# barronalex/Tacotron

Measured on AMD Instinct MI355X. Metric: mel-frames/sec (train step, batch=32 r=2), higher is better.
Workload: dtype f32

## Files before the change

### include/taco_hip.h

```cpp
#ifndef TACO_HIP_H
#define TACO_HIP_H

#include <stddef.h>
#include <stdint.h>

#ifdef __cplusplus
extern "C" {
#endif
#pragma GCC visibility push(default)

#define TACO_VERSION 120

#define TACO_OK 0
#define TACO_EINVAL (-1)
#define TACO_ELAUNCH (-2)
#define TACO_ENOTFOUND (-3)

#define TACO_ACT_NONE 0
#define TACO_ACT_RELU 1
#define TACO_ACT_SIGMOID 2
#define TACO_ACT_TANH 3

typedef struct TacoShape {
  int32_t B;
  int32_t Tt;
  int32_t Td;
  int32_t r;
  int32_t V;
  int32_t S;
} TacoShape;

typedef struct TacoTensorInfo {
  char name[64];
  int64_t offset;
  int64_t size;
  int32_t ndim;
  int32_t dims[4];
} TacoTensorInfo;

int taco_version(void);
const char* taco_last_error_string(void);

int64_t taco_param_count(const TacoShape* shape);
int taco_param_table(const TacoShape* shape, TacoTensorInfo* rows, int cap);

int64_t taco_workspace_bytes(const TacoShape* shape, int train);
int taco_workspace_table(const TacoShape* shape, int train, TacoTensorInfo* rows, int cap);

int taco_conv_gemm(const float* A, int lda, const float* W, int ldw, const float* bias, const float* scale,
                   const float* shift, const float* residual, int ldr, const uint8_t* keep, float* C, int ldc,
                   float* Cpre, int M, int N, int K, int taps, int T, int pad_l, int act, void* stream);

int taco_debug_gemm2_window(int lo, int hi);
int64_t taco_debug_weight_image(const float* W, int ldw, int taps, int K, int N, void* img, int64_t img_bytes, void* stream);
int taco_debug_conv_gemm_nld(const float* A, int lda, const float* W, int ldw, int nld, const float* bias, float* C, int ldc, int M,
                             int N, int K, int act, void* stream);
int taco_debug_conv_gemm_ksplit(const float* A, int lda, const float* W, int ldw, const float* bias, float* C, int ldc, int M,
                                int N, int K, int taps, int T, int pad_l, int act, float* slabs, int64_t slab_floats,
                                void* stream);

int taco_gemm_tn(const float* A, int lda, const float* dY, int ldy, float* dW, int ldw, int M, int N, int K, int taps,
                 int T, int pad_l, int accumulate, void* stream);

int taco_debug_gemm_naive(const float* A, int lda, const float* W, int ldw, const float* bias, float* C, int ldc,
                          int M, int N, int K, int taps, int T, int pad_l, int act, void* stream);

int taco_bigru_fwd(const float* x, const float* wg_fw, const float* bg_fw, const float* wc_fw, const float* bc_fw,
                   const float* wg_bw, const float* bg_bw, const float* wc_bw, const float* bc_bw, float* xg,
                   float* out, float* ruc, int B, int T, void* stream);

int taco_debug_bigru_rec_fwd(const float* xg, const float* wg_fw, const float* wc_fw, const float* wg_bw, const float* wc_bw,
                             const float* h0, float* out, float* ruc, int B, int T, void* stream);
int taco_debug_bigru_bwd(const float* dout, const float* out, const float* ruc, const float* wghT_fw, const float* wchT_fw,
                         const float* wghT_bw, const float* wchT_bw, const float* h0, float* dxg, float* rh, float* dh0, int B, int T,
                         void* stream);
int taco_debug_highway_stack_fwd(const float* x, const float* const* wt, const float* const* bt, const float* const* wh,
                                 const float* const* bh, float* const* th, float* const* y, const float* const* wa,
                                 const float* const* rowb, float* const* hx, int M, int nl, int T, void* stream);
int taco_debug_highway_stack_bwd(const float* g, const float* const* wT, const float* const* th, const float* const* x,
                                 float* const* dth, float* gout, const float* const* waT, float* const* dhx, int M, int nl, void* stream);
int taco_debug_prenet_fwd(const float* x, const float* w1, const float* b1, const float* w2, const float* b2, const uint8_t* keep1,
                          const uint8_t* keep2, float* y1, float* y2, int M, void* stream);
int taco_debug_prenet_bwd(const float* dy2, const float* w2T, const float* w1T, const uint8_t* keep1, const uint8_t* keep2,
                          const float* y1_in, const float* y2_in, float* dz2, float* dz1, float* dx, int M, void* stream);

int taco_debug_conv_bank_pool_fwd(const float* x, int lda, const float* const* W, const float* const* bias, const float* scale,
                                  const float* shift, float scale_mul, float* pool, float* bank, int ldc, int M, int T, int F, int N, int K,
                                  void* stream);
int taco_debug_conv_gemm_pool_bwd(const float* A, int lda, const float* W, int ldw, const float* pool_x, const float* scale,
                                  const float* shift, float scale_mul, float* C, int ldc, float* dgamma, float* dbeta, int M, int N, int K,
                                  int taps, int T, int pad_l, void* stream);
int taco_debug_bn_maxpool_fwd(const float* x, const float* gamma, const float* beta, float* y, int B, int T, int C, void* stream);
int taco_debug_bn_maxpool_bwd(const float* x, const float* gamma, const float* beta, const float* dy, float* dx, float* dgamma,
                              float* dbeta, int B, int T, int C, void* stream);
int taco_debug_bank_gather(const float* dbank, int lda, const float* const* WT, const float* residual, int ldr, float* dx_out, int ldc,
                           float* slabs, int64_t slab_floats, int M, int T, int F, int K, int N, int pad_l, int S, void* stream);
int taco_debug_conv_gemm_batch_atomic(const float* dbank, int lda, const float* const* WT, const float* residual, int ldr, float* dx_out,
                                      int ldc, int M, int T, int F, int K, int N, void* stream);
int taco_debug_conv_gemm_rowbias(const float* A, int lda, const float* W, int ldw, const float* rowb, int bias_stride, float* C, int ldc,
                                 int M, int T, int N, int K, void* stream);
int taco_debug_gemm_tn_group(int n, const float* const* A, const int* lda, const float* const* Y, const int* ldy, float* const* W,
                             const int* ldw, float* const* dbias, const int* M, const int* N, const int* K, const int* taps,
                             const int* T, const int* pad_l, void* stream);
int taco_debug_gemm_tn_strided(const float* A, int lda, int64_t strideA, const float* Y, int ldy, int64_t strideY, float* W, int ldw,
                               int64_t strideW, int M, int N, int K, int T, int pad_l, int batch, void* stream);

// ... 213 lines not shown
```

### tacotron_amd/csrc/gemm.hip

```cpp
#include <algorithm>

#include "bf16x3.h"
#include "common.h"
#include "kernels.h"

namespace {

constexpr int BK = 16;

__device__ __forceinline__ float4 sel4(bool ok, const float4 t) {
  return make_float4(ok ? t.x : 0.f, ok ? t.y : 0.f, ok ? t.z : 0.f, ok ? t.w : 0.f);
}

struct RowInfo {
  int m;
  int t;
  bool ok;
};

template <int WM, int WN, bool VA, bool VB>
__global__ __launch_bounds__(256) void conv_gemm_kernel(ConvGemmBatch batch) {
  constexpr int BM = 64 * WM, BN = 64 * WN;
  constexpr int LDS_A = BM + 4, LDS_B = BN + 4;
  constexpr int A_PER = BM / 64;
// ... 176 lines not shown
        for (int e = 0; e < 16; ++e) {
          const int m = min(mrow + (e & 3) + 8 * (e >> 2), P.M - 1);
          res_e[e] = P.residual[(int64_t)m * P.ldr + n];
        }
      }
      float pre_e[16];
#pragma unroll
      for (int e = 0; e < 16; ++e) {
        float v = apply_act(acc[i][j][e] + bias_e[e], P.act);
        if (P.keep) v = keep_e[e] ? v * 2.0f : 0.0f;
        pre_e[e] = v;
        if (P.scale || P.shift) v = v * sc + sf;
        acc[i][j][e] = v + res_e[e];
      }
      __builtin_amdgcn_sched_barrier(0);
#pragma unroll
      for (int e = 0; e < 16; ++e) {
        const int m = mrow + (e & 3) + 8 * (e >> 2);
        if (m >= P.M) continue;
        if (P.Cpre) P.Cpre[(int64_t)m * P.ldc + n] = pre_e[e];
        if (P.atomic_out) atomicAdd(&P.C[(int64_t)m * P.ldc + n], acc[i][j][e]);
        else P.C[(int64_t)m * P.ldc + n] = acc[i][j][e];
      }
    }
  }
}

__global__ void conv_gemm_tapsum_kernel(ConvGemmProblem P, const float* __restrict__ slabs, int taps) {
  const int64_t total4 = (int64_t)P.M * P.N / 4;
  const int64_t slab = (int64_t)P.M * P.N;
  for (int64_t i = (int64_t)blockIdx.x * blockDim.x + threadIdx.x; i < total4; i += (int64_t)gridDim.x * blockDim.x) {
    const int m = (int)(i * 4 / P.N), n0 = (int)(i * 4 - (int64_t)m * P.N);
    float4 s = reinterpret_cast<const float4*>(slabs)[i];
    for (int t = 1; t < taps; ++t) {
      const float4 v = reinterpret_cast<const float4*>(slabs + t * slab)[i];
      s.x += v.x; s.y += v.y; s.z += v.z; s.w += v.w;
    }
    float r[4] = {s.x, s.y, s.z, s.w};
#pragma unroll
    for (int j = 0; j < 4; ++j) {
      const int n = n0 + j;
      const float bias = P.bias ? (P.bias_stride ? P.bias[(int64_t)(m / P.T) * P.bias_stride + n] : P.bias[n]) : 0.f;
      float v = apply_act(r[j] + bias, P.act);
      if (P.keep) v = P.keep[(int64_t)m * P.N + n] ? v * 2.0f : 0.0f;
      if (P.Cpre) P.Cpre[(int64_t)m * P.ldc + n] = v;
      if (P.scale || P.shift) v = v * (P.scale ? P.scale[n] * P.scale_mul : 1.f) + (P.shift ? P.shift[n] : 0.f);
      if (P.residual) v += P.residual[(int64_t)m * P.ldr + n];
      if (P.atomic_out) P.C[(int64_t)m * P.ldc + n] += v;
      else P.C[(int64_t)m * P.ldc + n] = v;
    }
  }
}

template <int WM, int WN, bool VA, bool VB, bool BX = false>
__device__ __forceinline__ void gemm_tn_body(const GemmTnArgs& P, const int bx, const int by, const int bz_) {
  constexpr int BM = 64 * WM, BN = 64 * WN;
  constexpr int LDS_A = BM + 4, LDS_B = BN + 4;
  constexpr int A_PER = BM / 64, B_PER = BN / 64;
  const int k0 = bx * BM, n0 = by * BN;
  int z = bz_;
  const int split = z % P.splits;
  z /= P.splits;
  const int tap = z % P.taps;
  const int bz = z / P.taps;
  const float* A = P.A + (int64_t)bz * P.strideA;
  const float* Y = P.Y + (int64_t)bz * P.strideY;
  float* W = P.W + (int64_t)bz * P.strideW + (int64_t)tap * P.K * P.ldw;

  __shared__ __attribute__((aligned(16))) float As[2][BK][LDS_A];
  __shared__ __attribute__((aligned(16))) float Bs[2][BK][LDS_B];

  const int tid = threadIdx.x, lane = tid & 63, wave = tid >> 6;
  const int wm = wave >> 1, wn = wave & 1;
  const int sh = tap - P.pad_l;

  constexpr int A_COLS4 = BM / 4, B_COLS4 = BN / 4;
  constexpr int A_RSTEP = 256 / A_COLS4, B_RSTEP = 256 / B_COLS4;
  const int a_c4 = tid % A_COLS4, a_r = tid / A_COLS4;
  const int b_c4 = tid % B_COLS4, b_r = tid / B_COLS4;

  const int m_begin = split * P.chunk;
  const int m_end = min(P.M, m_begin + P.chunk);
  const int nit = (m_end - m_begin + BK - 1) / BK;
  if (nit <= 0) return;

  float4 ra[A_PER], rb[B_PER];
  const bool do_bias = P.dbias != nullptr && bx == 0 && tap == 0;
  float4 bsum[B_PER];
#pragma unroll
  for (int i = 0; i < B_PER; ++i) bsum[i] = make_float4(0.f, 0.f, 0.f, 0.f);
  constexpr int kOOB = (int)0x80000000;
  __amdgpu_buffer_rsrc_t rsA, rsY;
  int a_vo[A_PER], a_t[A_PER], b_vo[B_PER];
  int sh_t = sh;
  if constexpr (VA) {
    int kcol = k0 + a_c4 * 4;
    if (P.ktap > 0) {
      const int tc = kcol / P.ktap;
      kcol -= tc * P.ktap;
      sh_t = tc - P.pad_l;
    }
    rsA = __builtin_amdgcn_make_buffer_rsrc(const_cast<float*>(A - (int64_t)16 * P.lda), 0, 0x7fffffff, 0x00020000);
#pragma unroll
    for (int i = 0; i < A_PER; ++i) {
      const int r = a_r + i * A_RSTEP, k = k0 + a_c4 * 4;
      a_vo[i] = (r < BK && k < P.K) ? ((m_begin + r + sh_t + 16) * P.lda + kcol) * 4 : kOOB;
      a_t[i] = (m_begin + r) % P.T;
    }
  }
  if constexpr (VB) {
    rsY = __builtin_amdgcn_make_buffer_rsrc(const_cast<float*>(Y), 0, 0x7fffffff, 0x00020000);
#pragma unroll
    for (int i = 0; i < B_PER; ++i) {
      const int r = b_r + i * B_RSTEP, n = n0 + b_c4 * 4;
      b_vo[i] = (r < BK && n < P.Nld) ? ((m_begin + r) * P.ldy + n) * 4 : kOOB;
    }
  }
  auto as_f4 = [](auto v) { return __builtin_bit_cast(float4, v); };
  auto load_tile = [&](int it) {
    const int mm0 = m_begin + it * BK;
#pragma unroll
    for (int i = 0; i < A_PER; ++i) {
      float4 v = make_float4(0.f, 0.f, 0.f, 0.f);
      const int r = a_r + i * A_RSTEP;
      const int m = mm0 + r;
      const int k = k0 + a_c4 * 4;
      if constexpr (VA) {
        const bool ok = m < m_end && (unsigned)(a_t[i] + sh_t) < (unsigned)P.T;
        v = as_f4(__builtin_amdgcn_raw_buffer_load_b128(rsA, ok ? a_vo[i] : kOOB, it * (BK * 4) * P.lda, 0));
        a_t[i] += BK;
        if (P.T >= BK) a_t[i] = a_t[i] >= P.T ? a_t[i] - P.T : a_t[i];
        else a_t[i] %= P.T;
      } else if (r < BK && m < m_end) {
        const int st = (m % P.T) + sh;
        if (st >= 0 && st < P.T) {
          const float* p = A + (int64_t)(m + sh) * P.lda + k;
          if (k < P.K) v.x = p[0];
          if (k + 1 < P.K) v.y = p[1];
          if (k + 2 < P.K) v.z = p[2];
          if (k + 3 < P.K) v.w = p[3];
        }
      }
      ra[i] = v;
    }
#pragma unroll
    for (int i = 0; i < B_PER; ++i) {
      float4 v = make_float4(0.f, 0.f, 0.f, 0.f);
      const int r = b_r + i * B_RSTEP;
      const int m = mm0 + r;
      const int n = n0 + b_c4 * 4;
      if constexpr (VB) {
        v = as_f4(__builtin_amdgcn_raw_buffer_load_b128(rsY, m < m_end ? b_vo[i] : kOOB, it * (BK * 4) * P.ldy, 0));
      } else if (r < BK && m < m_end) {
        const float* p = Y + (int64_t)m * P.ldy + n;
        if (n < P.N) v.x = p[0];
        if (n + 1 < P.N) v.y = p[1];
        if (n + 2 < P.N) v.z = p[2];
        if (n + 3 < P.N) v.w = p[3];
      }
      rb[i] = v;
    }
  };
  auto store_tile = [&](int buf) {
#pragma unroll
    for (int i = 0; i < A_PER; ++i) {
      const int r = a_r + i * A_RSTEP;
      if (r < BK) *reinterpret_cast<float4*>(&As[buf][r][a_c4 * 4]) = ra[i];
    }
#pragma unroll
    for (int i = 0; i < B_PER; ++i) {
      const int r = b_r + i * B_RSTEP;
      const float4 v = rb[i];
      if (r < BK) *reinterpret_cast<float4*>(&Bs[buf][r][b_c4 * 4]) = v;
      if (do_bias) { bsum[i].x += v.x; bsum[i].y += v.y; bsum[i].z += v.z; bsum[i].w += v.w; }
    }
  };

  f32x16 acc[WM][WN];
#pragma unroll
  for (int i = 0; i < WM; ++i)
#pragma unroll
    for (int j = 0; j < WN; ++j)
#pragma unroll
      for (int e = 0; e < 16; ++e) acc[i][j][e] = 0.f;
  f32x16 acc_lo[BX ? WM : 1][BX ? WN : 1];
#pragma unroll
  for (int i = 0; i < (BX ? WM : 1); ++i)
#pragma unroll
    for (int j = 0; j < (BX ? WN : 1); ++j)
#pragma unroll
      for (int e = 0; e < 16; ++e) acc_lo[i][j][e] = 0.f;

  load_tile(0);
  store_tile(0);
  __syncthreads();
  const int lk = lane >> 5, li = lane & 31;
  for (int it = 0; it < nit; ++it) {
    const int buf = it & 1;
    if (it + 1 < nit) load_tile(it + 1);
    if constexpr (BX) {
      static_assert(BK == 16, "one v_mfma_f32_32x32x16_bf16 group per 16-row tile");
      Pl3 pa[WM], pb[WN];
#pragma unroll
      for (int i = 0; i < WM; ++i) {
        float f[8];
#pragma unroll
        for (int q = 0; q < 8; ++q) f[q] = As[buf][2 * q + lk][wm * (32 * WM) + i * 32 + li];
        pa[i] = split8(f[0], f[1], f[2], f[3], f[4], f[5], f[6], f[7]);
      }
#pragma unroll
      for (int j = 0; j < WN; ++j) {
        float f[8];
#pragma unroll
        for (int q = 0; q < 8; ++q) f[q] = Bs[buf][2 * q + lk][wn * (32 * WN) + j * 32 + li];
        pb[j] = split8(f[0], f[1], f[2], f[3], f[4], f[5], f[6], f[7]);
      }
#pragma unroll
      for (int i = 0; i < WM; ++i)
#pragma unroll
        for (int j = 0; j < WN; ++j) {
          mfma6_2(acc[i][j], acc_lo[i][j], pa[i], pb[j]);
        }
      if (it + 1 < nit) store_tile(buf ^ 1);
      __syncthreads();
      continue;
    }
    float a[2][WM], b[2][WN];
#pragma unroll
    for (int i = 0; i < WM; ++i) a[0][i] = As[buf][lk][wm * (32 * WM) + i * 32 + li];
#pragma unroll
    for (int j = 0; j < WN; ++j) b[0][j] = Bs[buf][lk][wn * (32 * WN) + j * 32 + li];
#pragma unroll
    for (int kk = 0; kk < BK; kk += 2) {
      const int cur = (kk >> 1) & 1, nxt = cur ^ 1;
      if (kk + 2 < BK) {
#pragma unroll
        for (int i = 0; i < WM; ++i) a[nxt][i] = As[buf][kk + 2 + lk][wm * (32 * WM) + i * 32 + li];
#pragma unroll
        for (int j = 0; j < WN; ++j) b[nxt][j] = Bs[buf][kk + 2 + lk][wn * (32 * WN) + j * 32 + li];
      }
#pragma unroll
      for (int i = 0; i < WM; ++i)
#pragma unroll
        for (int j = 0; j < WN; ++j)
          acc[i][j] = __builtin_amdgcn_mfma_f32_32x32x2f32(a[cur][i], b[cur][j], acc[i][j], 0, 0, 0);
    }
    if (it + 1 < nit) store_tile(buf ^ 1);
    __syncthreads();
  }

  if constexpr (BX) {
#pragma unroll
    for (int i = 0; i < WM; ++i)
#pragma unroll
      for (int j = 0; j < WN; ++j) acc[i][j] += acc_lo[i][j];
  }
#pragma unroll
  for (int i = 0; i < WM; ++i) {
#pragma unroll
    for (int j = 0; j < WN; ++j) {
      const int n = n0 + wn * (32 * WN) + j * 32 + li;
      if (n >= P.N) continue;
#pragma unroll
      for (int e = 0; e < 16; ++e) {
        const int k = k0 + wm * (32 * WM) + i * 32 + (e & 3) + 8 * (e >> 2) + 4 * lk;
        if (k >= P.K) continue;
        atomicAdd(&W[(int64_t)k * P.ldw + n], acc[i][j][e]);
      }
    }
  }
  if (do_bias) {
    float* cs = &As[0][0][0];
    float4 t = make_float4(0.f, 0.f, 0.f, 0.f);
#pragma unroll
    for (int i = 0; i < B_PER; ++i) { t.x += bsum[i].x; t.y += bsum[i].y; t.z += bsum[i].z; t.w += bsum[i].w; }
    __syncthreads();
    *reinterpret_cast<float4*>(&cs[b_r * LDS_B + b_c4 * 4]) = t;
    __syncthreads();
    float* db = P.dbias + (int64_t)bz * P.N;
    for (int i = tid; i < BN; i += 256) {
      float c = 0.f;
      for (int r = 0; r < B_RSTEP; ++r) c += cs[r * LDS_B + i];
      if (n0 + i < P.N) atomicAdd(&db[n0 + i], c);
    }
  }
}

__device__ __forceinline__ void tn_xcd_order(int L, int per, int gz, bool on, int& t, int& z) {
  const int zfull = gz & ~7;
  if (on && L < per * zfull) {
    const int x = L & 7, s = L >> 3;
    const int g = s / per;
    z = x + 8 * g;
    t = s - g * per;
  } else {
    z = L / per;
    t = L - z * per;
  }
}

template <int WM, int WN, bool VA, bool VB, bool BX = false>
__global__ __launch_bounds__(256) void gemm_tn_kernel(GemmTnArgs P) {
  const int gx = gridDim.x, per = gx * gridDim.y;
  int t, z;
  tn_xcd_order(blockIdx.x + gx * (blockIdx.y + gridDim.y * blockIdx.z), per, gridDim.z, P.xcd != 0, t, z);
  const int by = t / gx;
  gemm_tn_body<WM, WN, VA, VB, BX>(P, t - by * gx, by, z);
}

template <bool BX>
__global__ __launch_bounds__(256) void gemm_tn_batch_kernel(GemmTnBatch B) {
  int pi = 0;
  for (int i = 1; i < B.n; ++i)
    if ((int)blockIdx.x >= B.first[i]) pi = i;
  const GemmTnArgs& P = B.p[pi];
  const int rel = blockIdx.x - B.first[pi];
  const int gx = B.gx[pi], per = gx * B.gy[pi], gz = P.batch * P.taps * P.splits;
  if (rel >= per * gz) return;
  int t, z;
  tn_xcd_order(rel, per, gz, P.xcd != 0, t, z);
  const int by = t / gx;
  gemm_tn_body<1, 1, true, true, BX>(P, t - by * gx, by, z);
}

__global__ void gemm_naive_kernel(ConvGemmProblem P) {
  const int64_t idx = (int64_t)blockIdx.x * blockDim.x + threadIdx.x;
  if (idx >= (int64_t)P.M * P.N) return;
  const int m = (int)(idx / P.N), n = (int)(idx % P.N);
  const int t = m % P.T;
  float acc = 0.f;
  for (int tap = 0; tap < P.taps; ++tap) {
    const int st = t + tap - P.pad_l;
    if (st < 0 || st >= P.T) continue;
    const float* a = P.A + (int64_t)(m + tap - P.pad_l) * P.lda;
    const float* w = P.W + (int64_t)tap * P.K * P.ldw + n;
    for (int k = 0; k < P.K; ++k) acc = fmaf(a[k], w[(int64_t)k * P.ldw], acc);
  }
  if (P.bias) acc += P.bias[n];
  P.C[(int64_t)m * P.ldc + n] = apply_act(acc, P.act);
}

inline bool aligned16(const void* p) { return (reinterpret_cast<uintptr_t>(p) & 15) == 0; }

}

void conv_gemm_set_flags(ConvGemmProblem& p) {
  p.flags = 0;
  if (p.Nld <= 0) p.Nld = (p.N % 4 == 0) ? p.N : 0;
  if (p.lda % 4 == 0 && aligned16(p.A) && p.K % 4 == 0) p.flags |= 1;
  if (p.ldw % 4 == 0 && aligned16(p.W) && ((int64_t)p.K * p.ldw) % 4 == 0 && p.Nld > 0 && p.Nld % 4 == 0 && p.Nld <= p.ldw)
    p.flags |= 2;
}

template <int WM, int WN>
static void dispatch_nn(int flags, dim3 grid, hipStream_t s, ConvGemmBatch& batch) {
  switch (flags & 3) {
    case 3: TACO_KLAUNCH((conv_gemm_kernel<WM, WN, true, true>), grid, dim3(256), 0, s, batch); break;
    case 1: TACO_KLAUNCH((conv_gemm_kernel<WM, WN, true, false>), grid, dim3(256), 0, s, batch); break;
    case 2: TACO_KLAUNCH((conv_gemm_kernel<WM, WN, false, true>), grid, dim3(256), 0, s, batch); break;
    default: TACO_KLAUNCH((conv_gemm_kernel<WM, WN, false, false>), grid, dim3(256), 0, s, batch); break;
  }
}

int launch_conv_gemm_batch(ConvGemmBatch& batch, hipStream_t stream) {
  TACO_REQUIRE(batch.n >= 1 && batch.n <= kMaxGemmBatch, "conv_gemm: batch size %d out of range", batch.n);
  int maxM = 0, maxN = 0, flags = 3;
  double work = 0;
  for (int i = 0; i < batch.n; ++i) {
    ConvGemmProblem& p = batch.p[i];
    TACO_REQUIRE(p.A && p.W && p.C, "conv_gemm: null operand");
    TACO_REQUIRE(p.M > 0 && p.N > 0 && p.K > 0 && p.taps > 0 && p.T > 0, "conv_gemm: bad dims M=%d N=%d K=%d taps=%d T=%d",
                 p.M, p.N, p.K, p.taps, p.T);
    TACO_REQUIRE(p.M % p.T == 0, "conv_gemm: M (%d) must be a multiple of T (%d)", p.M, p.T);
    conv_gemm_set_flags(p);
    flags &= p.flags;
// ... 75 lines not shown
          ConvGemmProblem& r = b.p[c];
          r = ConvGemmProblem();
          r.A = p.A; r.lda = p.lda; r.W = p.W; r.ldw = p.ldw; r.Nld = p.Nld; r.C = slabs + c * mn; r.ldc = p.N;
          r.M = p.M; r.N = p.N; r.K = p.K; r.taps = p.taps; r.T = p.T; r.pad_l = p.pad_l; r.act = TACO_ACT_NONE;
          r.it0 = c * per;
          r.it1 = std::min(nit, (c + 1) * per);
          conv_gemm_set_flags(r);
        }
        const int pslot = taco_prof_begin(2, stream);
        taco_prof_label(2, pslot, "nn-ksplit S=%d M=%d N=%d K=%d taps=%d", bestS, p.M, p.N, p.K, p.taps);
        const int rc = launch_conv_gemm2(b, stream, true);
        if (rc == TACO_OK) {
          const int64_t total4 = mn / 4;
          const int grid = (int)((total4 + 255) / 256 > 2048 ? 2048 : (total4 + 255) / 256);
          TACO_KLAUNCH(conv_gemm_tapsum_kernel, dim3(grid), dim3(256), 0, stream, p, slabs, bestS);
          taco_prof_end(2, pslot, stream, 2.0 * p.M * p.N * p.K * p.taps);
          TACO_LAUNCH_CHECK("conv_gemm2 k-split");
          return TACO_OK;
        }
        taco_prof_cancel(2, pslot, stream);
        if (rc != TACO_ENOTFOUND) return rc;
      }
    }
  }
  const double tiles64 = (double)cdiv(p.M, 64) * cdiv(p.N, 64);
  if (!slabs || p.taps < 2 || p.taps > kMaxGemmBatch || p.N % 4 != 0 || p.atomic_out || tiles64 > 320 || p.K < 512)
    return launch_conv_gemm(p, stream);
  ConvGemmBatch b;
  b.n = p.taps;
  const int64_t slab = (int64_t)p.M * p.N;
  for (int t = 0; t < p.taps; ++t) {
    ConvGemmProblem q;
    q.A = p.A; q.lda = p.lda; q.W = p.W + (int64_t)t * p.K * p.ldw; q.ldw = p.ldw; q.Nld = p.Nld;
    q.C = slabs + t * slab; q.ldc = p.N;
    q.M = p.M; q.N = p.N; q.K = p.K; q.taps = 1; q.T = p.T; q.pad_l = p.pad_l - t;
    q.act = TACO_ACT_NONE;
    b.p[t] = q;
  }
  TACO_TRY(launch_conv_gemm_batch(b, stream));
  const int64_t total4 = slab / 4;
  const int grid = (int)((total4 + 255) / 256 > 2048 ? 2048 : (total4 + 255) / 256);
  TACO_KLAUNCH(conv_gemm_tapsum_kernel, dim3(grid), dim3(256), 0, stream, p, slabs, p.taps);
  TACO_LAUNCH_CHECK("conv_gemm_tapsum");
  return TACO_OK;
}

int launch_conv_gemm(const ConvGemmProblem& p, hipStream_t stream) {
  ConvGemmBatch b;
  b.n = 1;
  b.p[0] = p;
  return launch_conv_gemm_batch(b, stream);
}

template <int WM, int WN>
static void dispatch_tn(int flags, dim3 grid, hipStream_t s, const GemmTnArgs& a) {
  switch (flags & 3) {
    case 3:
      if (env_bf16x() && a.chunk <= bf16x_max_chain()) TACO_KLAUNCH((gemm_tn_kernel<WM, WN, true, true, true>), grid, dim3(256), 0, s, a);
      else TACO_KLAUNCH((gemm_tn_kernel<WM, WN, true, true>), grid, dim3(256), 0, s, a);
      break;
    case 1: TACO_KLAUNCH((gemm_tn_kernel<WM, WN, true, false>), grid, dim3(256), 0, s, a); break;
    case 2: TACO_KLAUNCH((gemm_tn_kernel<WM, WN, false, true>), grid, dim3(256), 0, s, a); break;
    default: TACO_KLAUNCH((gemm_tn_kernel<WM, WN, false, false>), grid, dim3(256), 0, s, a); break;
  }
}

static int tn_block_target() {
  const int x = sw_int<SW_TN_BLOCKS>();
  return x > 0 ? x : 3072;
}

static int plan_gemm_tn(GemmTnArgs& a, bool force_small, dim3& grid, int64_t group_tiles = 0) {
  a.flags = 0;
  if (a.Nld <= 0) a.Nld = (a.N % 4 == 0) ? a.N : 0;
  const int64_t lim31 = (int64_t)1 << 31;
  if (a.lda % 4 == 0 && aligned16(a.A) && a.strideA % 4 == 0 && a.K % 4 == 0 && ((int64_t)a.M + a.taps + 48) * a.lda * 4 < lim31)
    a.flags |= 1;
  if (a.ldy % 4 == 0 && aligned16(a.Y) && a.strideY % 4 == 0 && a.Nld > 0 && a.Nld % 4 == 0 && a.Nld <= a.ldy &&
      ((int64_t)a.M + 16) * a.ldy * 4 < lim31)
    a.flags |= 2;
  const bool merge_taps = sw_on<SW_TN_MERGE_TAPS>();
  if (merge_taps && a.ktap == 0 && (a.flags & 1) && a.taps > 1 && a.taps <= 17 && a.K % 64 != 0 && a.pad_l <= 16 && a.taps - 1 - a.pad_l <= 16) {
    a.ktap = a.K;
    a.K *= a.taps;
    a.taps = 1;
  }
  const int force_bm = sw_int<SW_TN_BM>(), big_tiles = sw_int<SW_TN_BIG_TILES>();
  bool big = !force_small && (int64_t)cdiv(a.K, 128) * cdiv(a.N, 128) * a.taps * a.batch >= big_tiles && a.K >= 128 && a.N >= 128;
  if (!force_small && force_bm == 128 && a.K >= 128 && a.N >= 128) big = true;
  if (force_bm == 64) big = false;
  const int bm = big ? 128 : 64;
  const int64_t tiles = (int64_t)cdiv(a.K, bm) * cdiv(a.N, bm) * a.taps * a.batch;
  const int64_t fill = group_tiles > tiles ? group_tiles : tiles;
  int splits = taco_deterministic() ? 1 : (int)((tn_block_target() + fill - 1) / fill);
  const int max_splits = a.M >= 1280 ? cdiv(a.M, 320) : cdiv(a.M, 64);
  if (splits > max_splits) splits = max_splits;
  if (splits < 1) splits = 1;
  int chunk = cdiv(a.M, splits);
  chunk = cdiv(chunk, BK) * BK;
  splits = cdiv(a.M, chunk);
  a.splits = splits;
  a.chunk = chunk;
  grid = dim3(cdiv(a.K, bm), cdiv(a.N, bm), a.batch * a.taps * splits);
  a.xcd = sw_int<SW_TN_XCD>();
  return bm;
}

int launch_gemm_tn(GemmTnArgs a, bool zero_first, hipStream_t stream) {
  TACO_REQUIRE(a.A && a.Y && a.W, "gemm_tn: null operand");
  TACO_REQUIRE(a.M > 0 && a.N > 0 && a.K > 0 && a.taps > 0 && a.T > 0 && a.batch > 0, "gemm_tn: bad dims");
  TACO_REQUIRE(a.M % a.T == 0, "gemm_tn: M (%d) must be a multiple of T (%d)", a.M, a.T);
  if (zero_first) {
// ... 30 lines not shown
  TACO_REQUIRE(b.n >= 0 && b.n <= kMaxTnBatch, "gemm_tn_batch: %d problems out of range", b.n);
  GemmTnBatch grouped;
  int blocks = 0;
  GemmTnArgs big[kMaxTnBatch];
  int nbig = 0;
  double big_flops = 0;
  int64_t group_tiles = 0;
  for (int i = 0; i < b.n; ++i) {
    dim3 grid;
    GemmTnArgs probe = b.p[i];
    if (probe.A && probe.M > 0 && probe.N > 0 && probe.K > 0 && probe.taps > 0 && probe.batch > 0 && !gemm_tn2_eligible(probe) &&
        plan_gemm_tn(probe, false, grid) == 64 && probe.flags == 3)
      group_tiles += (int64_t)grid.x * grid.y * probe.taps * probe.batch;
  }
  for (int i = 0; i < b.n; ++i) {
    GemmTnArgs a = b.p[i];
    TACO_REQUIRE(a.A && a.Y && a.W, "gemm_tn_batch: null operand");
    TACO_REQUIRE(a.M > 0 && a.N > 0 && a.K > 0 && a.taps > 0 && a.T > 0 && a.batch > 0 && a.M % a.T == 0, "gemm_tn_batch: bad dims");
    if (gemm_tn2_eligible(a)) {
      big[nbig++] = a;
      big_flops += 2.0 * a.M * a.N * a.K * a.taps;
      continue;
    }
    dim3 grid;
    GemmTnArgs probe = a;
    const int bm = plan_gemm_tn(probe, false, grid, group_tiles);
    if (bm == 128 || probe.flags != 3) {
      TACO_TRY(launch_gemm_tn(a, false, stream));
      continue;
    }
    const int j = grouped.n++;
    grouped.p[j] = probe;
    grouped.first[j] = blocks;
    grouped.gx[j] = (int)grid.x;
    grouped.gy[j] = (int)grid.y;
    blocks += (int)(grid.x * grid.y * grid.z);
    blocks = (blocks + 7) & ~7;
  }
  if (nbig > 0) {
    const int pslot = taco_prof_begin(2, stream);
    TACO_TRY(launch_gemm_tn2(big, nbig, stream));
    taco_prof_end(2, pslot, stream, big_flops);
    TACO_LAUNCH_CHECK("gemm_tn2 batch");
  }
  if (grouped.n > 0) {
    double flops = 0;
    for (int i = 0; i < grouped.n; ++i)
      flops += 2.0 * grouped.p[i].M * grouped.p[i].N * grouped.p[i].K * grouped.p[i].taps * grouped.p[i].batch;
    const int pslot = taco_prof_begin(2, stream);
    taco_prof_label(2, pslot, "tn-batch n=%d blocks=%d first: M=%d N=%d K=%d taps=%d", grouped.n, blocks, grouped.p[0].M, grouped.p[0].N, grouped.p[0].K,
                    grouped.p[0].taps);
    int max_chunk = 0;
    for (int i = 0; i < grouped.n; ++i) max_chunk = grouped.p[i].chunk > max_chunk ? grouped.p[i].chunk : max_chunk;
    if (env_bf16x() && max_chunk <= bf16x_max_chain()) TACO_KLAUNCH(gemm_tn_batch_kernel<true>, dim3(blocks), dim3(256), 0, stream, grouped);
    else TACO_KLAUNCH(gemm_tn_batch_kernel<false>, dim3(blocks), dim3(256), 0, stream, grouped);
    taco_prof_end(2, pslot, stream, flops);
    TACO_LAUNCH_CHECK("gemm_tn_batch");
  }
  b.n = 0;
  return TACO_OK;
}

int launch_gemm_naive(const ConvGemmProblem& p, hipStream_t stream) {
  const int64_t n = (int64_t)p.M * p.N;
  TACO_KLAUNCH(gemm_naive_kernel, dim3(cdiv(n, 256)), dim3(256), 0, stream, p);
  TACO_LAUNCH_CHECK("gemm_naive");
  return TACO_OK;
}


extern "C" int taco_debug_conv_gemm_batch_atomic(const float* dbank, int lda, const float* const* WT, const float* residual, int ldr,
                                                 float* dx_out, int ldc, int M, int T, int F, int K, int N, void* stream) {
  const char* who = "taco_debug_conv_gemm_batch_atomic";
  TACO_REQUIRE(M > 0 && M <= kDoorMaxRows, "%s: M must be in [1, 2^22], got %d", who, M);
  TACO_REQUIRE(T > 0 && M % T == 0, "%s: T must be positive and divide M = %d, got %d", who, M, T);
  TACO_REQUIRE(F >= 1 && F <= kMaxGemmBatch, "%s: F must be in [1, %d], got %d", who, kMaxGemmBatch, F);
  TACO_REQUIRE(N > 0 && N <= kDoorMaxCols, "%s: N must be in [1, 2^14], got %d", who, N);
  TACO_REQUIRE(K > 0 && K <= kDoorMaxCols, "%s: K must be in [1, 2^14], got %d", who, K);
  TACO_REQUIRE(lda >= F * K, "%s: lda must be >= F K = %d, got %d", who, F * K, lda);
  TACO_REQUIRE(ldc >= N, "%s: ldc must be >= N = %d, got %d", who, N, ldc);
  TACO_REQUIRE(!residual || ldr >= N, "%s: ldr must be >= N = %d, got %d", who, N, ldr);
  TACO_REQUIRE(WT, "%s: WT is null", who);
  DoorOperands o;
  o.in(dbank, door_span(M, (int64_t)F * K, lda), "dbank");
  for (int f = 1; f <= F; ++f) o.in(WT[f - 1], (size_t)f * K * N * sizeof(float), "WT[%d]", f - 1);
  o.in_opt(residual, door_span(M, N, ldr), "residual");
  o.out(dx_out, door_span(M, N, ldc), "dx_out");
  TACO_TRY(o.check(who));
  ConvGemmBatch batch;
  batch.n = F;
  for (int k = 1; k <= F; ++k) {
    ConvGemmProblem& p = batch.p[F - k];
    p = ConvGemmProblem();
    p.A = dbank + (k - 1) * K; p.lda = lda; p.W = WT[k - 1]; p.ldw = N; p.C = dx_out; p.ldc = ldc; p.M = M; p.N = N;
    p.K = K; p.taps = k; p.T = T; p.pad_l = (k - 1) - (k - 1) / 2; p.act = TACO_ACT_NONE; p.atomic_out = 1;
    if (k == 1) {
      p.residual = residual;
      p.ldr = ldr;
    }
  }
  return launch_conv_gemm_batch(batch, as_stream(stream));
}

extern "C" int taco_debug_conv_gemm_rowbias(const float* A, int lda, const float* W, int ldw, const float* rowb, int bias_stride, float* C,
                                            int ldc, int M, int T, int N, int K, void* stream) {
  const char* who = "taco_debug_conv_gemm_rowbias";
  TACO_REQUIRE(M > 0 && M <= kDoorMaxRows, "%s: M must be in [1, 2^22], got %d", who, M);
  TACO_REQUIRE(T > 0 && M % T == 0, "%s: T must be positive and divide M = %d, got %d", who, M, T);
// ... 82 lines not shown
```

### tacotron_amd/lib.py

```python
from __future__ import annotations

import collections
import ctypes as C
import math
import os

from . import QUEUES_SET_BY_USER as _QUEUES_SET_BY_USER, TORCH_IMPORTED_FIRST as _TORCH_IMPORTED_FIRST

import numpy as np
import torch

from .argcheck import (float_arg, int_arg, no_overlap, on_gpu, pow2_bins, step_q_arg, tensor_arg,
                       host_int32 as _host_int32, own_or_given as _own_or_given, unit_interval as _unit_interval)

HW_QUEUES_LATE = (not _QUEUES_SET_BY_USER) and (_TORCH_IMPORTED_FIRST or (torch.cuda.is_available() and torch.cuda.is_initialized()))


def effective_hw_queues() -> int:
    if HW_QUEUES_LATE:
        return 4
    try:
        return int(os.environ.get('GPU_MAX_HW_QUEUES', '4'))
    except ValueError:
        return 4

_HERE = os.path.dirname(os.path.abspath(__file__))
LIB_PATH = os.environ.get('TACO_LIB') or os.path.join(_HERE, 'libtaco_hip.so')


class TacoError(RuntimeError):
    pass


class TacoShape(C.Structure):
    _fields_ = [('B', C.c_int32), ('Tt', C.c_int32), ('Td', C.c_int32), ('r', C.c_int32), ('V', C.c_int32),
                ('S', C.c_int32)]

    def __repr__(self):
        return 'TacoShape(B=%d, Tt=%d, Td=%d, r=%d, V=%d, S=%d)' % (self.B, self.Tt, self.Td, self.r, self.V, self.S)


class TacoTensorInfo(C.Structure):
    _fields_ = [('name', C.c_char * 64), ('offset', C.c_int64), ('size', C.c_int64), ('ndim', C.c_int32),
                ('dims', C.c_int32 * 4)]


class TacoStopRule(C.Structure):
    _fields_ = [('end_offset', C.c_int32), ('hold', C.c_int32), ('min_steps', C.c_int32), ('reserved', C.c_int32)]

    def __init__(self, end_offset=1, hold=4, min_steps=8):
        super().__init__(int(end_offset), int(hold), int(min_steps), 0)

    def __repr__(self):
        return 'TacoStopRule(end_offset=%d, hold=%d, min_steps=%d)' % (self.end_offset, self.hold, self.min_steps)


if not os.path.exists(LIB_PATH):
    raise ImportError(
        'tacotron_amd: %s not found -- build it with `python -c "import __graft_entry__ as g; g.build()"` '
        '(or tacotron_amd/csrc/build.sh).  There is no CPU fallback.' % LIB_PATH)

_lib = C.CDLL(LIB_PATH)

_P = C.c_void_p
_I = C.c_int
_SH = C.POINTER(TacoShape)
_INT_MAX = (1 << 31) - 1

EXPORTS = {
    'taco_version': (C.c_int, []),
    'taco_last_error_string': (C.c_char_p, []),
    'taco_param_count': (C.c_int64, [_SH]),
    'taco_param_table': (C.c_int, [_SH, C.POINTER(TacoTensorInfo), _I]),
    'taco_workspace_bytes': (C.c_int64, [_SH, _I]),
    'taco_workspace_table': (C.c_int, [_SH, _I, C.POINTER(TacoTensorInfo), _I]),
    'taco_conv_gemm': (C.c_int, [_P, _I, _P, _I, _P, _P, _P, _P, _I, _P, _P, _I, _P, _I, _I, _I, _I, _I, _I, _I, _P]),
    'taco_debug_gemm2_window': (C.c_int, [_I, _I]),
    'taco_debug_weight_image': (C.c_int64, [_P, _I, _I, _I, _I, _P, C.c_int64, _P]),
    'taco_debug_conv_gemm_nld': (C.c_int, [_P, _I, _P, _I, _I, _P, _P, _I, _I, _I, _I, _I, _P]),
    'taco_debug_conv_gemm_ksplit': (C.c_int, [_P, _I, _P, _I, _P, _P, _I, _I, _I, _I, _I, _I, _I, _I, _P, C.c_int64, _P]),
    'taco_gemm_tn': (C.c_int, [_P, _I, _P, _I, _P, _I, _I, _I, _I, _I, _I, _I, _I, _P]),
    'taco_debug_gemm_naive': (C.c_int, [_P, _I, _P, _I, _P, _P, _I, _I, _I, _I, _I, _I, _I, _I, _P]),
    'taco_bigru_fwd': (C.c_int, [_P] * 12 + [_I, _I, _P]),
    'taco_debug_bigru_rec_fwd': (C.c_int, [_P] * 8 + [_I, _I, _P]),
    'taco_debug_bigru_bwd': (C.c_int, [_P] * 11 + [_I, _I, _P]),
    'taco_debug_highway_stack_fwd': (C.c_int, [_P] * 10 + [_I, _I, _I, _P]),
    'taco_debug_highway_stack_bwd': (C.c_int, [_P] * 8 + [_I, _I, _P]),
    'taco_debug_prenet_fwd': (C.c_int, [_P] * 9 + [_I, _P]),
    'taco_debug_prenet_bwd': (C.c_int, [_P] * 10 + [_I, _P]),
    'taco_debug_conv_bank_pool_fwd': (C.c_int, [_P, _I, _P, _P, _P, _P, C.c_float, _P, _P, _I, _I, _I, _I, _I, _I, _P]),
    'taco_debug_conv_gemm_pool_bwd': (C.c_int, [_P, _I, _P, _I, _P, _P, _P, C.c_float, _P, _I, _P, _P, _I, _I, _I, _I, _I, _I, _P]),
    'taco_debug_bn_maxpool_fwd': (C.c_int, [_P] * 4 + [_I, _I, _I, _P]),
    'taco_debug_bn_maxpool_bwd': (C.c_int, [_P] * 7 + [_I, _I, _I, _P]),
    'taco_debug_bank_gather': (C.c_int, [_P, _I, _P, _P, _I, _P, _I, _P, C.c_int64, _I, _I, _I, _I, _I, _I, _I, _P]),
    'taco_debug_conv_gemm_batch_atomic': (C.c_int, [_P, _I, _P, _P, _I, _P, _I, _I, _I, _I, _I, _I, _P]),
    'taco_debug_conv_gemm_rowbias': (C.c_int, [_P, _I, _P, _I, _P, _I, _P, _I, _I, _I, _I, _I, _P]),
    'taco_debug_gemm_tn_group': (C.c_int, [_I] + [_P] * 13 + [_P]),
    'taco_debug_gemm_tn_strided': (C.c_int, [_P, _I, C.c_int64, _P, _I, C.c_int64, _P, _I, C.c_int64, _I, _I, _I, _I, _I, _I, _P]),
    'taco_debug_embedding': (C.c_int, [_P, _P, _P, _I, _I, _I, _P]),
    'taco_debug_embedding_bwd': (C.c_int, [_P, _P, _P, _I, _I, _I, _P]),
    'taco_debug_highway_combine': (C.c_int, [_P, _P, _P, _I, _P]),
    'taco_debug_highway_combine_bwd': (C.c_int, [_P] * 5 + [_I, _P]),
    'taco_debug_act_bwd': (C.c_int, [_P, _P, _P, _P, C.c_int64, _I, _P]),
    'taco_debug_affine_act_bwd': (C.c_int, [_P] * 6 + [_I, _I, _I, _P]),
    'taco_debug_colsum_batched': (C.c_int, [_P, _I, _P, _I, _I, _I, _P]),
    'taco_debug_mask_rows': (C.c_int, [_P, _P, _P, _I, _I, _I, _P]),
    'taco_debug_center_rows': (C.c_int, [_P, _P, _P, _I, _I, _I, _P]),
    'taco_debug_mask_pos': (C.c_int, [_P, _I, _P, _I, _I, _I, C.c_float, _P]),
    'taco_debug_zero_tail_rows': (C.c_int, [_P, _I, _P, _I, _P, _I, _I, _P]),
    'taco_debug_add': (C.c_int, [_P, _P, _P, C.c_int64, _P]),
    'taco_debug_l1_loss': (C.c_int, [_P, _P, _P, _I, _I, _I, _P, _P, _P, _I, _I, _I, _P, _P, _P, _P]),
    'taco_debug_transpose_batch': (C.c_int, [_I] + [_P] * 7 + [_P]),
    'taco_debug_sumsq': (C.c_int, [_P, C.c_int64, _P, _P]),
    'taco_forward': (C.c_int, [_SH] + [_P] * 17),
    'taco_backward': (C.c_int, [_SH] + [_P] * 14),
    'taco_infer': (C.c_int, [_SH] + [_P] * 9),
    'taco_infer_stop': (C.c_int, [_SH, _P, _P, _P, _P, C.POINTER(TacoStopRule), _P, _P, _P, _P, _P, _P]),
    'taco_alignment_scores': (C.c_int, [_P, _P, _P, _I, _P, _P, _I, _I, _I, _P]),
    'taco_alignment_path_workspace_bytes': (C.c_int64, [_I, _I, _I]),
    'taco_alignment_path': (C.c_int, [_P, _P, _P, _I, _P, _P, _P, _P, _P, _I, _I, _I, _P]),
    'taco_frames_active': (C.c_int, [_P, C.c_float, _P, _I, _I, _I, _P]),
    'taco_frame_dtw_workspace_bytes': (C.c_int64, [_I, _I, _I, _I]),
    'taco_frame_dtw': (C.c_int, [_P, _P, _P, _P, _P, _P, _P, _P, _I, _I, _I, _I, _I, _P]),
    'taco_frame_dtw_path_workspace_bytes': (C.c_int64, [_I, _I, _I, _I]),
    'taco_frame_dtw_path': (C.c_int, [_P, _P, _P, _P, _P, _P, _P, _P, _P, _P, _I, _I, _I, _I, _I, _P]),
    'taco_path_f0_scores': (C.c_int, [_P, _P, _P, _P, _P, C.c_float, _P, _P, _I, _I, _I, _P]),
    'taco_clip_adam_step': (C.c_int, [_P, _P, _P, _P, C.c_int64, C.c_float, C.c_float, C.c_int64, _P, _P, _P]),
    'taco_clip_adam_step_guarded': (C.c_int, [_P, _P, _P, _P, C.c_int64, C.c_float, C.c_float, C.c_int64, _P, _P, _P, _P]),
    'taco_clear_error': (C.c_int, [_SH, _I, _P, _P]),
    'taco_grad_segments': (C.c_int, [_SH, C.POINTER(C.c_int64)]),
# ... 78 lines not shown

def make_shape(B, Tt, Td, r, V, S=1) -> TacoShape:
    return TacoShape(int(B), int(Tt), int(Td), int(r), int(V), int(S))


def version() -> int:
    return _lib.taco_version()


def _size(fn_name, *args) -> int:
    n = getattr(_lib, fn_name)(*[C.byref(a) if isinstance(a, TacoShape) else int(a) for a in args])
    if n < 0:
        raise TacoError('%s(%s): bad arguments (rc=%d)' % (fn_name, ', '.join(repr(a) for a in args), n))
    return n


def param_count(shape: TacoShape) -> int:
    return _size('taco_param_count', shape)


def _table(fn, *args):
    n = fn(*args, None, 0)
    if n < 0:
        raise TacoError(last_error())
    rows = (TacoTensorInfo * n)()
    fn(*args, rows, n)
    return [(r.name.decode(), int(r.offset), int(r.size), tuple(r.dims[i] for i in range(r.ndim))) for r in rows]


def param_table(shape: TacoShape):
    return _table(_lib.taco_param_table, C.byref(shape))


def workspace_bytes(shape: TacoShape, train: bool) -> int:
    return _size('taco_workspace_bytes', shape, train)


def workspace_table(shape: TacoShape, train: bool):
    return _table(_lib.taco_workspace_table, C.byref(shape), int(train))


def conv_gemm(A, W, C_out, M, N, K, taps=1, T=None, pad_l=0, act=0, bias=None, scale=None, shift=None, residual=None,
              keep=None, Cpre=None, lda=None, ldw=None, ldc=None, ldr=None):
    T = M if T is None else T
    _check(_lib.taco_conv_gemm(ptr(A), lda or K, ptr(W), ldw or N, ptr(bias), ptr(scale), ptr(shift), ptr(residual),
                               ldr or N, ptr(keep), ptr(C_out), ldc or N, ptr(Cpre), M, N, K, taps, T, pad_l, act,
                               stream_ptr()), 'taco_conv_gemm')


def debug_gemm2_window(lo, hi):
    return int(_lib.taco_debug_gemm2_window(lo, hi))


def conv_gemm_nld(A, W, C_out, M, N, K, nld, ldw, ldc, act=0, bias=None):
    _check(_lib.taco_debug_conv_gemm_nld(ptr(A), K, ptr(W), ldw, nld, ptr(bias), ptr(C_out), ldc, M, N, K, act, stream_ptr()),
           'taco_debug_conv_gemm_nld')


def conv_gemm_ksplit(A, W, C_out, M, N, K, slabs, taps=1, T=None, pad_l=0, act=0, bias=None):
    T = M if T is None else T
    _check(_lib.taco_debug_conv_gemm_ksplit(ptr(A), K, ptr(W), N, ptr(bias), ptr(C_out), N, M, N, K, taps, T, pad_l, act,
                                            ptr(slabs), slabs.numel(), stream_ptr()), 'taco_debug_conv_gemm_ksplit')


def gemm_tn(A, dY, dW, M, N, K, taps=1, T=None, pad_l=0, accumulate=False, lda=None, ldy=None, ldw=None):
    T = M if T is None else T
    _check(_lib.taco_gemm_tn(ptr(A), lda or K, ptr(dY), ldy or N, ptr(dW), ldw or N, M, N, K, taps, T, pad_l,
                             int(accumulate), stream_ptr()), 'taco_gemm_tn')


def weight_image_bytes(W, taps, K, N, ldw=None):
    need = _lib.taco_debug_weight_image(ptr(W), ldw or N, taps, K, N, None, 0, None)
    if need < 0:
        raise TacoError('taco_debug_weight_image: %d' % need)
    return int(need)


def weight_image(W=None, taps=1, K=0, N=0, ldw=None, img=None):
    if W is None:
        return int(_lib.taco_debug_weight_image(None, 0, 0, 0, 0, None, 0, None))
    ldw = ldw or N
    need = _lib.taco_debug_weight_image(ptr(W), ldw, taps, K, N, None, 0, None)
    if need < 0:
        raise TacoError('taco_debug_weight_image: %d' % need)
    if img is None:
        img = torch.empty(need // 2, dtype=torch.int16, device=W.device)
    assert img.numel() * img.element_size() >= need and img.data_ptr() % 16 == 0, 'taco: weight image buffer too small or misaligned'
    rc = _lib.taco_debug_weight_image(ptr(W), ldw, taps, K, N, ptr(img), need, stream_ptr())
    _check(int(rc), 'taco_debug_weight_image')
    return img


def debug_gemm_naive(A, W, C_out, M, N, K, taps=1, T=None, pad_l=0, act=0, bias=None):
    T = M if T is None else T
    _check(_lib.taco_debug_gemm_naive(ptr(A), K, ptr(W), N, ptr(bias), ptr(C_out), N, M, N, K, taps, T, pad_l, act,
                                      stream_ptr()), 'taco_debug_gemm_naive')


def bigru_fwd(x, w, xg, out, ruc, B, T):
    _check(_lib.taco_bigru_fwd(ptr(x), ptr(w['fw/gates/kernel']), ptr(w['fw/gates/bias']),
                               ptr(w['fw/candidate/kernel']), ptr(w['fw/candidate/bias']),
                               ptr(w['bw/gates/kernel']), ptr(w['bw/gates/bias']),
                               ptr(w['bw/candidate/kernel']), ptr(w['bw/candidate/bias']),
                               ptr(xg), ptr(out), ptr(ruc), B, T, stream_ptr()), 'taco_bigru_fwd')


# ... 1787 lines not shown
```

Baseline: 1.690 million.

## Store bf16x3 plane images in LDS for gemm_tn and read with transpose loads

In the bf16x3 weight-gradient GEMM, each tile is now split into hi/mid/lo bf16 planes once, when it is written to shared memory, using a row-interleaved, XOR-swizzled layout. The MFMA operands are then fetched with ds_read_tr16_b64 transpose reads. Before, every wave read eight scalar floats per operand and split them into planes each iteration. This removes the redundant per-wave split arithmetic and the strided scalar LDS reads, at the cost of extra shared memory for the plane buffers, which could lower occupancy. The path is on by default and has a debug toggle.

```diff
diff --git a/include/taco_hip.h b/include/taco_hip.h
--- a/include/taco_hip.h
+++ b/include/taco_hip.h
@@ -52,6 +52,7 @@
                    float* Cpre, int M, int N, int K, int taps, int T, int pad_l, int act, void* stream);
 
 int taco_debug_gemm2_window(int lo, int hi);
+int taco_debug_tn_planes(int on);
 int64_t taco_debug_weight_image(const float* W, int ldw, int taps, int K, int N, void* img, int64_t img_bytes, void* stream);
 int taco_debug_conv_gemm_nld(const float* A, int lda, const float* W, int ldw, int nld, const float* bias, float* C, int ldc, int M,
                              int N, int K, int act, void* stream);
diff --git a/tacotron_amd/csrc/gemm.hip b/tacotron_amd/csrc/gemm.hip
--- a/tacotron_amd/csrc/gemm.hip
+++ b/tacotron_amd/csrc/gemm.hip
@@ -252,7 +252,7 @@
   }
 }
 
-template <int WM, int WN, bool VA, bool VB, bool BX = false>
+template <int WM, int WN, bool VA, bool VB, bool BX = false, bool PL = false>
 __device__ __forceinline__ void gemm_tn_body(const GemmTnArgs& P, const int bx, const int by, const int bz_) {
   constexpr int BM = 64 * WM, BN = 64 * WN;
   constexpr int LDS_A = BM + 4, LDS_B = BN + 4;
@@ -267,8 +267,12 @@
   const float* Y = P.Y + (int64_t)bz * P.strideY;
   float* W = P.W + (int64_t)bz * P.strideW + (int64_t)tap * P.K * P.ldw;
 
+  static_assert(!PL || BX, "plane images are a form of the bf16x3 branch");
   __shared__ __attribute__((aligned(16))) float As[2][BK][LDS_A];
   __shared__ __attribute__((aligned(16))) float Bs[2][BK][LDS_B];
+  constexpr int PA_E = BM, PB_E = BN;
+  __shared__ __attribute__((aligned(16))) unsigned short Pa[2][3][BK][PA_E];
+  __shared__ __attribute__((aligned(16))) unsigned short Pb[2][3][BK][PB_E];
 
   const int tid = threadIdx.x, lane = tid & 63, wave = tid >> 6;
   const int wm = wave >> 1, wn = wave & 1;
@@ -361,17 +365,32 @@
       rb[i] = v;
     }
   };
+  static_assert(!PL || (A_RSTEP * A_PER == BK && B_RSTEP * B_PER == BK), "PL: the 256 threads' float4 cover exactly the 16 tile rows");
+  auto pl_row = [](int m) { return 8 * (m & 1) + (m >> 1); };
+  auto pl_swz = [](int r, int cols) { return cols == 64 ? (r >> 1) & 1 : r & 3; };
+  auto store_planes = [](const float4& v, unsigned short* h, unsigned short* m, unsigned short* l) {
+    unsigned h0, m0, l0, h1, m1, l1;
+    split2(v.x, v.y, h0, m0, l0);
+    split2(v.z, v.w, h1, m1, l1);
+    *reinterpret_cast<uint2*>(h) = make_uint2(h0, h1);
+    *reinterpret_cast<uint2*>(m) = make_uint2(m0, m1);
+    *reinterpret_cast<uint2*>(l) = make_uint2(l0, l1);
+  };
   auto store_tile = [&](int buf) {
 #pragma unroll
     for (int i = 0; i < A_PER; ++i) {
       const int r = a_r + i * A_RSTEP;
-      if (r < BK) *reinterpret_cast<float4*>(&As[buf][r][a_c4 * 4]) = ra[i];
+      const int ir = pl_row(r), ic = (a_c4 * 4) ^ (32 * pl_swz(ir, BM));
+      if constexpr (PL) store_planes(ra[i], &Pa[buf][0][ir][ic], &Pa[buf][1][ir][ic], &Pa[buf][2][ir][ic]);
+      else if (r < BK) *reinterpret_cast<float4*>(&As[buf][r][a_c4 * 4]) = ra[i];
     }
 #pragma unroll
     for (int i = 0; i < B_PER; ++i) {
       const int r = b_r + i * B_RSTEP;
       const float4 v = rb[i];
-      if (r < BK) *reinterpret_cast<float4*>(&Bs[buf][r][b_c4 * 4]) = v;
+      const int ir = pl_row(r), ic = (b_c4 * 4) ^ (32 * pl_swz(ir, BN));
+      if constexpr (PL) store_planes(v, &Pb[buf][0][ir][ic], &Pb[buf][1][ir][ic], &Pb[buf][2][ir][ic]);
+      else if (r < BK) *reinterpret_cast<float4*>(&Bs[buf][r][b_c4 * 4]) = v;
       if (do_bias) { bsum[i].x += v.x; bsum[i].y += v.y; bsum[i].z += v.z; bsum[i].w += v.w; }
     }
   };
@@ -395,26 +414,36 @@
   store_tile(0);
   __syncthreads();
   const int lk = lane >> 5, li = lane & 31;
+  const int pl_lane_r = 8 * lk + ((lane >> 2) & 3), pl_lane_c = (lane & 16) + 4 * (lane & 3);
+  auto read_planes = [&](auto& img, int col0, int cols) {
+    const int c = (col0 + pl_lane_c) ^ (32 * pl_swz(pl_lane_r, cols));
+    typedef short s16x4 __attribute__((ext_vector_type(4)));
+    typedef unsigned u32x2 __attribute__((ext_vector_type(2)));
+    u32x4 w[3];
+#pragma unroll
+    for (int pl = 0; pl < 3; ++pl) {
+      u32x2 half[2];
+#pragma unroll
+      for (int rd = 0; rd < 2; ++rd)
+        half[rd] = __builtin_bit_cast(u32x2, __builtin_amdgcn_ds_read_tr16_b64_v4i16(
+                                                 (__attribute__((address_space(3))) s16x4*)&img[pl][pl_lane_r + 4 * rd][c]));
+      w[pl] = u32x4{half[0].x, half[0].y, half[1].x, half[1].y};
+    }
+    Pl3 p;
+    p.h = w[0]; p.m = w[1]; p.l = w[2];
+    return p;
+  };
   for (int it = 0; it < nit; ++it) {
     const int buf = it & 1;
     if (it + 1 < nit) load_tile(it + 1);
-    if constexpr (BX) {
+    if constexpr (BX && PL) {
       static_assert(BK == 16, "one v_mfma_f32_32x32x16_bf16 group per 16-row tile");
       Pl3 pa[WM], pb[WN];
 #pragma unroll
-      for (int i = 0; i < WM; ++i) {
-        float f[8];
-#pragma unroll
-        for (int q = 0; q < 8; ++q) f[q] = As[buf][2 * q + lk][wm * (32 * WM) + i * 32 + li];
-        pa[i] = split8(f[0], f[1], f[2], f[3], f[4], f[5], f[6], f[7]);
-      }
-#pragma unroll
-      for (int j = 0; j < WN; ++j) {
-        float f[8];
-#pragma unroll
-        for (int q = 0; q < 8; ++q) f[q] = Bs[buf][2 * q + lk][wn * (32 * WN) + j * 32 + li];
-        pb[j] = split8(f[0], f[1], f[2], f[3], f[4], f[5], f[6], f[7]);
-      }
+      for (int i = 0; i < WM; ++i) pa[i] = read_planes(Pa[buf], wm * (32 * WM) + i * 32, BM);
+#pragma unroll
+      for (int j = 0; j < WN; ++j) pb[j] = read_planes(Pb[buf], wn * (32 * WN) + j * 32, BN);
+      __builtin_amdgcn_sched_barrier(0);
 #pragma unroll
       for (int i = 0; i < WM; ++i)
 #pragma unroll
@@ -424,6 +453,32 @@
       if (it + 1 < nit) store_tile(buf ^ 1);
       __syncthreads();
       continue;
+    } else if constexpr (BX) {
+      static_assert(BK == 16, "one v_mfma_f32_32x32x16_bf16 group per 16-row tile");
+      Pl3 pa[WM], pb[WN];
+#pragma unroll
+      for (int i = 0; i < WM; ++i) {
+        float f[8];
+#pragma unroll
+        for (int q = 0; q < 8; ++q) f[q] = As[buf][2 * q + lk][wm * (32 * WM) + i * 32 + li];
+        pa[i] = split8(f[0], f[1], f[2], f[3], f[4], f[5], f[6], f[7]);
+      }
+#pragma unroll
+      for (int j = 0; j < WN; ++j) {
+        float f[8];
+#pragma unroll
+        for (int q = 0; q < 8; ++q) f[q] = Bs[buf][2 * q + lk][wn * (32 * WN) + j * 32 + li];
+        pb[j] = split8(f[0], f[1], f[2], f[3], f[4], f[5], f[6], f[7]);
+      }
+#pragma unroll
+      for (int i = 0; i < WM; ++i)
+#pragma unroll
+        for (int j = 0; j < WN; ++j) {
+          mfma6_2(acc[i][j], acc_lo[i][j], pa[i], pb[j]);
+        }
+      if (it + 1 < nit) store_tile(buf ^ 1);
+      __syncthreads();
+      continue;
     }
     float a[2][WM], b[2][WN];
 #pragma unroll
@@ -470,7 +525,7 @@
     }
   }
   if (do_bias) {
-    float* cs = &As[0][0][0];
+    float* cs = PL ? reinterpret_cast<float*>(&Pa[0][0][0][0]) : &As[0][0][0];
     float4 t = make_float4(0.f, 0.f, 0.f, 0.f);
 #pragma unroll
     for (int i = 0; i < B_PER; ++i) { t.x += bsum[i].x; t.y += bsum[i].y; t.z += bsum[i].z; t.w += bsum[i].w; }
@@ -499,16 +554,16 @@
   }
 }
 
-template <int WM, int WN, bool VA, bool VB, bool BX = false>
+template <int WM, int WN, bool VA, bool VB, bool BX = false, bool PL = false>
 __global__ __launch_bounds__(256) void gemm_tn_kernel(GemmTnArgs P) {
   const int gx = gridDim.x, per = gx * gridDim.y;
   int t, z;
   tn_xcd_order(blockIdx.x + gx * (blockIdx.y + gridDim.y * blockIdx.z), per, gridDim.z, P.xcd != 0, t, z);
   const int by = t / gx;
-  gemm_tn_body<WM, WN, VA, VB, BX>(P, t - by * gx, by, z);
-}
-
-template <bool BX>
+  gemm_tn_body<WM, WN, VA, VB, BX, PL>(P, t - by * gx, by, z);
+}
+
+template <bool BX, bool PL = false>
 __global__ __launch_bounds__(256) void gemm_tn_batch_kernel(GemmTnBatch B) {
   int pi = 0;
   for (int i = 1; i < B.n; ++i)
@@ -520,7 +575,7 @@
   int t, z;
   tn_xcd_order(rel, per, gz, P.xcd != 0, t, z);
   const int by = t / gx;
-  gemm_tn_body<1, 1, true, true, BX>(P, t - by * gx, by, z);
+  gemm_tn_body<1, 1, true, true, BX, PL>(P, t - by * gx, by, z);
 }
 
 __global__ void gemm_naive_kernel(ConvGemmProblem P) {
@@ -702,12 +757,22 @@
   return launch_conv_gemm_batch(b, stream);
 }
 
+static int g_tn_planes = 1;
+static bool env_tn_planes() { return g_tn_planes != 0; }
+extern "C" int taco_debug_tn_planes(int on) {
+  const int was = g_tn_planes;
+  if (on >= 0) g_tn_planes = on != 0;
+  return was;
+}
+
 template <int WM, int WN>
 static void dispatch_tn(int flags, dim3 grid, hipStream_t s, const GemmTnArgs& a) {
   switch (flags & 3) {
     case 3:
-      if (env_bf16x() && a.chunk <= bf16x_max_chain()) TACO_KLAUNCH((gemm_tn_kernel<WM, WN, true, true, true>), grid, dim3(256), 0, s, a);
-      else TACO_KLAUNCH((gemm_tn_kernel<WM, WN, true, true>), grid, dim3(256), 0, s, a);
+      if (env_bf16x() && a.chunk <= bf16x_max_chain()) {
+        if (env_tn_planes()) TACO_KLAUNCH((gemm_tn_kernel<WM, WN, true, true, true, true>), grid, dim3(256), 0, s, a);
+        else TACO_KLAUNCH((gemm_tn_kernel<WM, WN, true, true, true>), grid, dim3(256), 0, s, a);
+      } else TACO_KLAUNCH((gemm_tn_kernel<WM, WN, true, true>), grid, dim3(256), 0, s, a);
       break;
     case 1: TACO_KLAUNCH((gemm_tn_kernel<WM, WN, true, false>), grid, dim3(256), 0, s, a); break;
     case 2: TACO_KLAUNCH((gemm_tn_kernel<WM, WN, false, true>), grid, dim3(256), 0, s, a); break;
@@ -844,8 +909,10 @@
                     grouped.p[0].taps);
     int max_chunk = 0;
     for (int i = 0; i < grouped.n; ++i) max_chunk = grouped.p[i].chunk > max_chunk ? grouped.p[i].chunk : max_chunk;
-    if (env_bf16x() && max_chunk <= bf16x_max_chain()) TACO_KLAUNCH(gemm_tn_batch_kernel<true>, dim3(blocks), dim3(256), 0, stream, grouped);
-    else TACO_KLAUNCH(gemm_tn_batch_kernel<false>, dim3(blocks), dim3(256), 0, stream, grouped);
+    if (env_bf16x() && max_chunk <= bf16x_max_chain()) {
+      if (env_tn_planes()) TACO_KLAUNCH((gemm_tn_batch_kernel<true, true>), dim3(blocks), dim3(256), 0, stream, grouped);
+      else TACO_KLAUNCH(gemm_tn_batch_kernel<true>, dim3(blocks), dim3(256), 0, stream, grouped);
+    } else TACO_KLAUNCH(gemm_tn_batch_kernel<false>, dim3(blocks), dim3(256), 0, stream, grouped);
     taco_prof_end(2, pslot, stream, flops);
     TACO_LAUNCH_CHECK("gemm_tn_batch");
   }
diff --git a/tacotron_amd/lib.py b/tacotron_amd/lib.py
--- a/tacotron_amd/lib.py
+++ b/tacotron_amd/lib.py
@@ -76,6 +76,7 @@
     'taco_workspace_table': (C.c_int, [_SH, _I, C.POINTER(TacoTensorInfo), _I]),
     'taco_conv_gemm': (C.c_int, [_P, _I, _P, _I, _P, _P, _P, _P, _I, _P, _P, _I, _P, _I, _I, _I, _I, _I, _I, _I, _P]),
     'taco_debug_gemm2_window': (C.c_int, [_I, _I]),
+    'taco_debug_tn_planes': (C.c_int, [_I]),
     'taco_debug_weight_image': (C.c_int64, [_P, _I, _I, _I, _I, _P, C.c_int64, _P]),
     'taco_debug_conv_gemm_nld': (C.c_int, [_P, _I, _P, _I, _I, _P, _P, _I, _I, _I, _I, _I, _P]),
     'taco_debug_conv_gemm_ksplit': (C.c_int, [_P, _I, _P, _I, _P, _P, _I, _I, _I, _I, _I, _I, _I, _I, _P, C.c_int64, _P]),
@@ -260,6 +261,10 @@
     return int(_lib.taco_debug_gemm2_window(lo, hi))
 
 
+def debug_tn_planes(on):
+    return int(_lib.taco_debug_tn_planes(int(on)))
+
+
 def conv_gemm_nld(A, W, C_out, M, N, K, nld, ldw, ldc, act=0, bias=None):
     _check(_lib.taco_debug_conv_gemm_nld(ptr(A), K, ptr(W), ldw, nld, ptr(bias), ptr(C_out), ldc, M, N, K, act, stream_ptr()),
            'taco_debug_conv_gemm_nld')
```

Result: no change. 1.703 million (median of 6 runs) (+0.8%).
